# 2Retr0/GodotGaussianSplatting

Measured on NVIDIA H100. Metric: Msplats/s, higher is better.
Workload: dtype f32

## Files before the change

godotgaussiansplatting_b200/csrc/common.cuh:

```cuda
#pragma once
#include <cuda_runtime.h>
#include <stdint.h>
#include <stdio.h>

#include "../../include/gsr.h"

namespace gsr {

constexpr int TILE = 16;
constexpr int NUM_PLANES = 15;
constexpr int PROJ_THREADS = 256;

void set_last_error(const char *fmt, ...);

#define GSR_CUDA_TRY(expr)                                                                         \
    do {                                                                                           \
        cudaError_t _e = (expr);                                                                   \
        if (_e != cudaSuccess) {                                                                   \
            ::gsr::set_last_error("%s:%d: %s -> %s", __FILE__, __LINE__, #expr, cudaGetErrorString(_e)); \
            return (_e == cudaErrorMemoryAllocation) ? GSR_ERR_OOM : GSR_ERR_CUDA;                 \
        }                                                                                          \
    } while (0)

__device__ __forceinline__ float g_max(float x, float y) { return (x < y) ? y : x; }
// ... 38 lines not shown
__device__ __forceinline__ float det_pow(float x, float y) {
    if (!(x > 0.0f)) return 0.0f;
    return det_exp2(__fmul_rn(y, det_log2(x)));
}

struct FrameState {
    unsigned long long dup_total;
    uint32_t dup_sorted;
    uint32_t visible;
    int32_t last_tile_plus1;
    uint32_t overflow;
    uint32_t proj_ticket;
    uint32_t pad0;
    unsigned long long staged;
    uint32_t comp_head;
    uint32_t comp_cta_limit;
    uint32_t pad[4];
};
static_assert(sizeof(FrameState) == 64, "FrameState is one 64-byte slot of the history ring");

struct Uniforms {
    float camera_pos[3];
    float model_scale;
    int32_t dims[2];
    float time;
    float pad;
};
static_assert(sizeof(Uniforms) == 32, "uniform block must be 32 bytes");

struct SortWorkspace {
    uint32_t *hist = nullptr;
    uint32_t *status = nullptr;
    uint32_t *tickets = nullptr;
    uint32_t *alt_keys = nullptr;
    uint32_t *alt_vals = nullptr;
    uint32_t *n_dev = nullptr;
    uint64_t max_n = 0;
    uint32_t max_tiles = 0;
    int grid_hist = 0, grid_sweep_pairs = 0, grid_sweep_keys = 0;
    size_t bytes() const;
};
int sort_workspace_create(SortWorkspace &ws, uint64_t max_n, bool need_alt_buffers);
void sort_workspace_destroy(SortWorkspace &ws);
int sort_pairs_device(SortWorkspace &ws, uint32_t *keys, uint32_t *vals, const uint32_t *n_ptr, uint32_t *alt_keys,
                      uint32_t *alt_vals, cudaStream_t stream, int *launches);
uint32_t sort_tile_keys();

struct ProjectionArgs {
    const float4 *soa;
    uint64_t plane_stride;
    uint32_t num_splats;
    float vp[32];
    Uniforms u;
    float focal_base[2];
    float lim_lo[2], lim_hi[2];
    int32_t band_y0, band_y1;
    int32_t row_mod, row_rem;
    int32_t fast_reject;
    int32_t sh_bulk_min;
    int32_t fast_mode;
    float w_frob2;
    float4 *records;
    uint32_t *keys, *values;
    uint32_t capacity;
    unsigned long long *lookback;
    FrameState *frame;
};
int launch_projection(const ProjectionArgs &a, cudaStream_t stream);

constexpr int INSTANCE_FRAME_FLOATS = 32;
constexpr int INSTANCE_XFORM_FLOATS = 24;
struct InstanceDesc {
    uint64_t first;
    uint32_t count;
    uint32_t warp0;
};
struct InstanceArgs {
    const float *frame;
// ... 101 lines not shown
```

godotgaussiansplatting_b200/csrc/gsr_api.cu:

```cuda
#include <math.h>
#include <stdarg.h>
#include <stdlib.h>
#include <stddef.h>
#include <string.h>
#include <unistd.h>

#include <new>

#include "common.cuh"

namespace gsr {

static thread_local char g_last_error[512] = "";

void set_last_error(const char *fmt, ...) {
    va_list ap;
    va_start(ap, fmt);
    vsnprintf(g_last_error, sizeof g_last_error, fmt, ap);
    va_end(ap);
}

}

using namespace gsr;

constexpr int EV_PER_FRAME = 7;

struct gsr_ctx {
    int device = 0;
    uint32_t flags = 0;
    uint64_t max_splats = 0, capacity = 0, plane_stride = 0, num_splats = 0;
    uint64_t cap_stride = 0;
    cudaStream_t stream = nullptr, own_stream = nullptr;
    float4 *soa = nullptr;
    float4 *records = nullptr;
    float4 *records2 = nullptr;
    uint32_t *keys = nullptr;
    uint32_t *vals = nullptr;
    uint32_t *keys_cur = nullptr, *vals_cur = nullptr;
    float4 *records_cur = nullptr;
    cudaStream_t front_stream = nullptr;
    cudaEvent_t front_gate = nullptr;
    int overlap = -1;
    SortWorkspace sort;
    FrameState *ring = nullptr;
    FrameState *frame = nullptr;
    unsigned long long *lookback = nullptr;
    uint32_t lookback_blocks = 0;
    uint64_t frame_counter = 0;
    uint2 *bounds = nullptr;
    uint32_t *comp_order = nullptr, *comp_hint = nullptr;
    int comp_ctas_per_sm = 2, comp_order_mode = 1, comp_max_ctas = 1, comp_sparse_per_sm = 5;
    uint64_t comp_hint_key = 0;
    FrameState *pick_frame = nullptr;
    ulonglong4 *trace = nullptr;
    uint32_t *trace_count = nullptr;
    uint32_t trace_cap = 0;
    float4 *fb = nullptr, *fb_ext = nullptr;
    const float *scene_depth = nullptr;
    float *depth_out = nullptr;
    float4 *pick_strip = nullptr;
    float4 *fb2 = nullptr;
    void *stage[2] = {nullptr, nullptr};
    float4 *fb_last = nullptr;
    cudaStream_t copy_stream = nullptr;
    cudaEvent_t ev_done[2] = {nullptr, nullptr}, ev_copied[2] = {nullptr, nullptr};
    bool copied_valid[2] = {false, false};
    uint64_t async_counter = 0;
    bool peer_mode = false, peer_opened = false;
    float4 *peer_fb[2] = {nullptr, nullptr};
    uint64_t peer_counter = 0;
// ... 71 lines not shown
        return GSR_ERR_CUDA;
    }
    if (device < 0 || device >= count) {
        set_last_error("device ordinal %d out of range [0,%d)", device, count);
        return GSR_ERR_INVALID;
    }
    cudaDeviceProp prop;
    GSR_CUDA_TRY(cudaGetDeviceProperties(&prop, device));
    if (prop.major != 9 || prop.minor != 0) {
        set_last_error("device %d is sm_%d%d; libgsr is built for sm_90a only", device, prop.major, prop.minor);
        return GSR_ERR_CUDA;
    }
    return GSR_OK;
}

void group_detach(gsr_ctx *c) {
    if (c->front_stream) cudaStreamSynchronize(c->front_stream);
    if (c->stream) cudaStreamSynchronize(c->stream);
    if (c->copy_stream) cudaStreamSynchronize(c->copy_stream);
    for (int i = 0; i < c->grp.n_opened; ++i) cudaIpcCloseMemHandle(c->grp.opened[i]);
    c->grp.n_opened = 0;
    if (c->grp.world > 1) { c->row_mod = 1; c->row_rem = 0; }
    c->grp.world = 0; c->grp.rank = 0; c->grp.seq = 0; c->grp.present_rows = 0;
    c->grp.root_fb[0] = c->grp.root_fb[1] = nullptr;
}

float4 *framebuffer(gsr_ctx *c) { return c->fb_ext ? c->fb_ext : (c->fb_last ? c->fb_last : c->fb); }

void free_ctx(gsr_ctx *c) {
    if (!c) return;
    cudaSetDevice(c->device);
    if (c->stream) cudaStreamSynchronize(c->stream);
    if (c->front_stream) { cudaStreamSynchronize(c->front_stream); cudaStreamDestroy(c->front_stream); }
    cudaFree(c->soa); cudaFree(c->records); cudaFree(c->records2); cudaFree(c->keys); cudaFree(c->vals);
    sort_workspace_destroy(c->sort);
    if (c->copy_stream) cudaStreamSynchronize(c->copy_stream);
    if (c->peer_opened) { cudaIpcCloseMemHandle(c->peer_fb[0]); cudaIpcCloseMemHandle(c->peer_fb[1]); }
    cudaFree(c->stage[0]); cudaFree(c->stage[1]);
    cudaFree(c->ring); cudaFree(c->lookback); cudaFree(c->bounds); cudaFree(c->comp_order); cudaFree(c->comp_hint); cudaFree(c->pick_frame); cudaFree(c->fb); cudaFree(c->fb2); cudaFree(c->pick); cudaFree(c->staging); cudaFree(c->pick_strip);
    for (int i = 0; i < 2; ++i) { if (c->ev_done[i]) cudaEventDestroy(c->ev_done[i]); if (c->ev_copied[i]) cudaEventDestroy(c->ev_copied[i]); }
    if (c->copy_stream) cudaStreamDestroy(c->copy_stream);
    cudaFree(c->sync_word);
    for (int i = 0; i < c->grp.n_opened; ++i) cudaIpcCloseMemHandle(c->grp.opened[i]);
    cudaFree(c->grp.arena);
    cudaFree(c->unsorted_keys); cudaFree(c->unsorted_vals); cudaFree(c->trace); cudaFree(c->trace_count);
    cudaFree(c->inst.desc); cudaFree(c->inst.warps); cudaFree(c->inst.frame);
    if (c->inst.ring) cudaFreeHost(c->inst.ring);
    for (int i = 0; i < GSR_INSTANCE_RING; ++i) if (c->inst.ev[i]) cudaEventDestroy(c->inst.ev[i]);
    delete[] c->inst.range; delete[] c->inst.xf;
    if (c->ev) {
        for (int i = 0; i < GSR_HISTORY_FRAMES * EV_PER_FRAME; ++i) if (c->ev[i]) cudaEventDestroy(c->ev[i]);
        delete[] c->ev;
    }
    if (c->ev_stat) {
        for (int i = 0; i < GSR_HISTORY_FRAMES; ++i) if (c->ev_stat[i]) cudaEventDestroy(c->ev_stat[i]);
        delete[] c->ev_stat;
    }
    if (c->host_ring) cudaFreeHost(c->host_ring);
    if (c->own_stream) cudaStreamDestroy(c->own_stream);
    delete c;
}

}

extern "C" {

GSR_API const char *gsr_error_string(int code) {
// ... 40 lines not shown
#define TRY_ALLOC(ptr, bytes)                                                                      \
    do {                                                                                           \
        cudaError_t _e = cudaMalloc((void **)&(ptr), (bytes));                                     \
        if (_e != cudaSuccess) {                                                                   \
            set_last_error("cudaMalloc(%s, %llu B) -> %s", #ptr, (unsigned long long)(bytes), cudaGetErrorString(_e)); \
            free_ctx(c);                                                                           \
            return _e == cudaErrorMemoryAllocation ? GSR_ERR_OOM : GSR_ERR_CUDA;                   \
        }                                                                                          \
    } while (0)

    cudaError_t se;
    {
        int least = 0, greatest = 0;
        cudaDeviceGetStreamPriorityRange(&least, &greatest);
        se = cudaStreamCreateWithPriority(&c->own_stream, cudaStreamNonBlocking, greatest);
    }
    if (se != cudaSuccess) { set_last_error("cudaStreamCreate -> %s", cudaGetErrorString(se)); free_ctx(c); return GSR_ERR_CUDA; }
    c->stream = c->own_stream;
    se = cudaStreamCreateWithFlags(&c->copy_stream, cudaStreamNonBlocking);
    if (se == cudaSuccess) {
        int least = 0, greatest = 0;
        cudaDeviceGetStreamPriorityRange(&least, &greatest);
        se = cudaStreamCreateWithPriority(&c->front_stream, cudaStreamNonBlocking, least);
    }
    for (int i = 0; i < 2 && se == cudaSuccess; ++i) {
        se = cudaEventCreateWithFlags(&c->ev_done[i], cudaEventDisableTiming);
        if (se == cudaSuccess) se = cudaEventCreateWithFlags(&c->ev_copied[i], cudaEventDisableTiming);
    }
    if (se != cudaSuccess) { set_last_error("copy stream/events -> %s", cudaGetErrorString(se)); free_ctx(c); return GSR_ERR_CUDA; }
    TRY_ALLOC(c->soa, sizeof(float4) * NUM_PLANES * c->plane_stride);
    TRY_ALLOC(c->records, sizeof(float4) * 3ull * c->max_splats);
    TRY_ALLOC(c->records2, sizeof(float4) * 3ull * c->max_splats);
    c->cap_stride = (c->capacity + 1023ull) & ~1023ull;
    TRY_ALLOC(c->keys, sizeof(uint32_t) * 3ull * c->cap_stride);
    TRY_ALLOC(c->vals, sizeof(uint32_t) * 3ull * c->cap_stride);
    c->keys_cur = c->keys; c->vals_cur = c->vals; c->records_cur = c->records;
    c->rec_entries = c->max_splats;
    c->lookback_blocks = projection_num_blocks((uint32_t)c->max_splats);
    c->lookback_cap = c->lookback_blocks;
    TRY_ALLOC(c->ring, sizeof(FrameState) * GSR_HISTORY_FRAMES);
    TRY_ALLOC(c->lookback, sizeof(unsigned long long) * ((size_t)c->lookback_blocks + 2u * GROUP_MAX * GROUP_MAX));
    c->frame = c->ring;
    TRY_ALLOC(c->pick, sizeof(float4));
    TRY_ALLOC(c->sync_word, sizeof(int32_t));
    c->staging_splats = c->max_splats < (1ull << 18) ? c->max_splats : (1ull << 18);
    TRY_ALLOC(c->staging, sizeof(float4) * NUM_PLANES * c->staging_splats);
#undef TRY_ALLOC
    rc = sort_workspace_create(c->sort, c->capacity, false);
    if (rc) { free_ctx(c); return rc; }
    c->ev = new (std::nothrow) cudaEvent_t[GSR_HISTORY_FRAMES * EV_PER_FRAME]();
    if (!c->ev) { free_ctx(c); return GSR_ERR_OOM; }
    for (int i = 0; i < GSR_HISTORY_FRAMES * EV_PER_FRAME; ++i) {
        if (cudaEventCreate(&c->ev[i]) != cudaSuccess) { set_last_error("cudaEventCreate failed"); free_ctx(c); return GSR_ERR_CUDA; }
    }
    c->ev_stat = new (std::nothrow) cudaEvent_t[GSR_HISTORY_FRAMES]();
    if (!c->ev_stat) { free_ctx(c); return GSR_ERR_OOM; }
    for (int i = 0; i < GSR_HISTORY_FRAMES; ++i) {
        if (cudaEventCreateWithFlags(&c->ev_stat[i], cudaEventDisableTiming) != cudaSuccess) { set_last_error("cudaEventCreate failed"); free_ctx(c); return GSR_ERR_CUDA; }
    }
    if (cudaHostAlloc((void **)&c->host_ring, sizeof(FrameState) * GSR_HISTORY_FRAMES, cudaHostAllocMapped | cudaHostAllocPortable) != cudaSuccess) {
        set_last_error("cudaHostAlloc(frame mirror) failed"); c->host_ring = nullptr; free_ctx(c); return GSR_ERR_OOM;
    }
    memset(c->host_ring, 0, sizeof(FrameState) * GSR_HISTORY_FRAMES);
    cudaMemsetAsync(c->soa, 0, sizeof(float4) * NUM_PLANES * c->plane_stride, c->stream);
    cudaMemsetAsync(c->records, 0, sizeof(float4) * 3ull * c->max_splats, c->stream);
    cudaMemsetAsync(c->records2, 0, sizeof(float4) * 3ull * c->max_splats, c->stream);
    cudaMemsetAsync(c->pick, 0, sizeof(float4), c->stream);
    cudaMemsetAsync(c->sync_word, 0, sizeof(int32_t), c->stream);
    cudaMemsetAsync(c->ring, 0, sizeof(FrameState) * GSR_HISTORY_FRAMES, c->stream);
// ... 139 lines not shown
        const float tfi0 = view_proj[16 + 0], tfi1 = view_proj[16 + 5];
        const volatile float hw = (float)u.dims[0] * 0.5f, hh = (float)u.dims[1] * 0.5f;
        const volatile float f0 = hw * tfi0, f1 = hh * tfi1;
        const volatile float t0 = 1.0f / tfi0, t1 = 1.0f / tfi1;
        const volatile float n0 = -t0, n1 = -t1;
        pa.focal_base[0] = f0; pa.focal_base[1] = f1;
        pa.lim_lo[0] = n0 * 1.3f; pa.lim_lo[1] = n1 * 1.3f;
        pa.lim_hi[0] = t0 * 1.3f; pa.lim_hi[1] = t1 * 1.3f;
    }
    {
        float g[3][3];
        for (int i = 0; i < 3; ++i)
            for (int j = 0; j < 3; ++j) {
                g[i][j] = 0.0f;
                for (int r = 0; r < 3; ++r) g[i][j] += view_proj[4 * i + r] * view_proj[4 * j + r];
            }
        float nrm = 0.0f;
        for (int i = 0; i < 3; ++i) {
            float row = 0.0f;
            for (int j = 0; j < 3; ++j) row += g[i][j] < 0.0f ? -g[i][j] : g[i][j];
            nrm = row > nrm ? row : nrm;
        }
        pa.w_frob2 = nrm * 1.0001f;
    }
}

static int grow_capacity(gsr_ctx *c, uint64_t want) {
    if (want > c->capacity_max) want = c->capacity_max;
    if (want <= c->capacity) return GSR_OK;
    GSR_CUDA_TRY(cudaStreamSynchronize(c->front_stream));
    GSR_CUDA_TRY(cudaStreamSynchronize(c->stream));
    GSR_CUDA_TRY(cudaStreamSynchronize(c->copy_stream));
    c->front_gate = nullptr;
    cudaFree(c->keys); cudaFree(c->vals); c->keys = c->vals = c->keys_cur = c->vals_cur = nullptr;
    sort_workspace_destroy(c->sort);
    const bool unsorted = c->unsorted_keys != nullptr;
    cudaFree(c->unsorted_keys); cudaFree(c->unsorted_vals); c->unsorted_keys = c->unsorted_vals = nullptr;
    c->capacity = want;
    c->cap_stride = (c->capacity + 1023ull) & ~1023ull;
    GSR_CUDA_TRY(cudaMalloc((void **)&c->keys, sizeof(uint32_t) * 3ull * c->cap_stride));
    GSR_CUDA_TRY(cudaMalloc((void **)&c->vals, sizeof(uint32_t) * 3ull * c->cap_stride));
    c->keys_cur = c->keys; c->vals_cur = c->vals;
    if (unsorted) {
        GSR_CUDA_TRY(cudaMalloc((void **)&c->unsorted_keys, sizeof(uint32_t) * c->capacity));
        GSR_CUDA_TRY(cudaMalloc((void **)&c->unsorted_vals, sizeof(uint32_t) * c->capacity));
    }
    return sort_workspace_create(c->sort, c->capacity, false);
}

static int track_capacity(gsr_ctx *c) {
    if (c->flags & GSR_FLAG_STATIC_CAPACITY) return GSR_OK;
    while (c->stats_polled < c->frame_counter) {
        if (c->frame_counter - c->stats_polled > GSR_HISTORY_FRAMES) { c->stats_polled = c->frame_counter - GSR_HISTORY_FRAMES; continue; }
        const uint32_t slot = (uint32_t)(c->stats_polled % GSR_HISTORY_FRAMES);
        if (cudaEventQuery(c->ev_stat[slot]) != cudaSuccess) { cudaGetLastError(); break; }
        const uint64_t m = c->host_ring[slot].dup_total;
        if (m > c->m_high) c->m_high = m;
        c->stats_polled += 1;
    }
    if (c->m_high * 2ull > c->capacity && c->capacity < c->capacity_max) return grow_capacity(c, c->m_high * 3ull);
    return GSR_OK;
}

struct GroupFrame { uint32_t seq; int parity; int rows_local; };

static int stage_times(gsr_ctx *c, uint32_t slot, float out[5], float *front_ms) {
    cudaEvent_t *ev = c->ev + EV_PER_FRAME * slot;
    float front = 0.f, recv = 0.f;
    GSR_CUDA_TRY(cudaEventElapsedTime(&front, ev[0], ev[1]));
    GSR_CUDA_TRY(cudaEventElapsedTime(&recv, ev[2], ev[3]));
    out[0] = front + recv;
    for (int i = 1; i < 4; ++i) GSR_CUDA_TRY(cudaEventElapsedTime(&out[i], ev[2 + i], ev[3 + i]));
    out[4] = out[0] + out[1] + out[2] + out[3];
    if (front_ms) *front_ms = front;
    return GSR_OK;
// ... 4 lines not shown
static size_t arena_records_off(uint64_t cap, uint64_t max_splats, int parity) { return GROUP_FLAGS_BYTES + sizeof(uint32_t) * cap * 2 * GROUP_PHASES + sizeof(float4) * 3ull * max_splats * (size_t)parity; }
static size_t arena_bytes(uint64_t cap, uint64_t max_splats) { return arena_records_off(cap, max_splats, GROUP_PHASES); }

static GroupPeers group_peers(const gsr_ctx *c, int parity) {
    (void)parity;
    GroupPeers p;
    memset(&p, 0, sizeof p);
    p.world = c->grp.world; p.rank = c->grp.rank;
    for (int r = 0; r < c->grp.world; ++r) p.flags[r] = c->grp.flags[r];
    return p;
}

static int render_enqueue(gsr_ctx *c, const float *view_proj, const void *uniforms32, float heatmap_factor, float4 *target = nullptr,
                          const GroupFrame *gf = nullptr) {
    if (!c || !view_proj || !uniforms32) return GSR_ERR_INVALID;
    if (c->width == 0) { set_last_error("gsr_render before gsr_resize"); return GSR_ERR_STATE; }
    Uniforms u;
    memcpy(&u, uniforms32, sizeof u);
    if (u.dims[0] != c->width || u.dims[1] != c->height) {
        set_last_error("uniform dims %dx%d differ from gsr_resize %dx%d", u.dims[0], u.dims[1], c->width, c->height);
        return GSR_ERR_INVALID;
    }
    int rc = use_device(c->device);
    if (rc) return rc;
    if ((rc = track_capacity(c))) return rc;
    cudaStream_t s = c->stream;
    const bool overlap = c->overlap > 0 && c->front_stream != nullptr;
    cudaStream_t fs = overlap ? c->front_stream : s;
    int launches = 0;
    const uint32_t slot = (uint32_t)(c->frame_counter % GSR_HISTORY_FRAMES);
    c->frame = c->ring + slot;
    cudaEvent_t *ev = c->ev + EV_PER_FRAME * slot;
    const int half = (int)(c->frame_counter & 1u);
    uint32_t *keys_in = c->keys + (size_t)half * c->cap_stride, *vals_in = c->vals + (size_t)half * c->cap_stride;
    uint32_t *keys_alt = c->keys + 2ull * c->cap_stride, *vals_alt = c->vals + 2ull * c->cap_stride;
    float4 *records = half ? c->records2 : c->records;
    const uint32_t n_tiles = (uint32_t)(c->tiles_x * c->tiles_y);

    if (overlap && c->front_gate) GSR_CUDA_TRY(cudaStreamWaitEvent(fs, c->front_gate, 0));
    const bool inst = c->inst.n > 0 && !gf;
    {
        uint32_t links = projection_num_blocks((uint32_t)(inst ? c->inst.drawn : c->max_splats));
        if (gf) {
            const uint64_t first = (uint64_t)c->grp.rank * c->grp.slice;
            const uint64_t count = first < c->max_splats ? ((c->max_splats - first) < c->grp.slice ? (c->max_splats - first) : c->grp.slice) : 0;
            links = projection_scatter_blocks((uint32_t)count) * (uint32_t)c->grp.world;
        }
        if ((rc = launch_frame_clear(c->frame, c->lookback, links, overlap ? nullptr : c->bounds, overlap ? 0u : n_tiles, fs))) return rc;
        launches += 1;
    }
    GSR_CUDA_TRY(cudaEventRecord(ev[0], fs));
    if (inst) {
        const uint32_t rs = (uint32_t)(c->inst.seq % GSR_INSTANCE_RING);
        if (c->inst.ev_used[rs] && cudaEventQuery(c->inst.ev[rs]) != cudaSuccess) {
            cudaGetLastError();
            GSR_CUDA_TRY(cudaEventSynchronize(c->inst.ev[rs]));
        }
        const size_t per = (size_t)c->inst.cap * INSTANCE_XFORM_FLOATS;
        memcpy(c->inst.ring + rs * per, c->inst.xf, sizeof(float) * INSTANCE_XFORM_FLOATS * c->inst.n);
        if ((rc = launch_instance_prepare(c->inst.ring_dev + rs * per, view_proj, u.camera_pos, c->inst.n,
                                          c->inst.frame + (size_t)half * c->inst.cap * INSTANCE_FRAME_FLOATS, fs))) return rc;
        GSR_CUDA_TRY(cudaEventRecord(c->inst.ev[rs], fs));
        c->inst.ev_used[rs] = true;
        c->inst.seq += 1;
        launches += 1;
    }

    ProjectionArgs pa;
// ... 36 lines not shown
        if ((rc = launch_projection_instanced(pa, ia, fs))) return rc;
        launches += pa.num_splats ? 1 : 0;
    } else {
        if ((rc = launch_projection(pa, fs))) return rc;
        launches += pa.num_splats ? 1 : 0;
    }
    GSR_CUDA_TRY(cudaEventRecord(ev[1], fs));

    if (overlap) {
        GSR_CUDA_TRY(cudaStreamWaitEvent(s, ev[1], 0));
        if ((rc = launch_frame_clear(nullptr, nullptr, 0u, c->bounds, n_tiles, s))) return rc;
        launches += 1;
    }
    GSR_CUDA_TRY(cudaEventRecord(ev[2], s));
    if (gf) {
        const int G = c->grp.world;
        char *mine = c->grp.peer_arena[c->grp.rank];
        if ((rc = launch_group_wait_segments(c->grp.flags[c->grp.rank], gf->parity, G, gf->seq, c->grp.seg_cap, (uint32_t)c->capacity, c->frame, s))) return rc;
        if ((rc = launch_gather_segments(c->grp.flags[c->grp.rank], G, c->grp.seg_cap,
                                         reinterpret_cast<const uint32_t *>(mine + arena_rx_keys_off(c->grp.rx_capacity, gf->parity)),
                                         reinterpret_cast<const uint32_t *>(mine + arena_rx_vals_off(c->grp.rx_capacity, gf->parity)), keys_in, vals_in,
                                         c->sm_count * 8, s))) return rc;
        records = reinterpret_cast<float4 *>(mine + arena_records_off(c->grp.rx_capacity, c->max_splats, gf->parity));
        launches += 2;
    }
    c->keys_cur = keys_in; c->vals_cur = vals_in; c->records_cur = records;
    GSR_CUDA_TRY(cudaEventRecord(ev[3], s));

    if (c->keep_unsorted) {
        GSR_CUDA_TRY(cudaMemcpyAsync(c->unsorted_keys, keys_in, sizeof(uint32_t) * c->capacity, cudaMemcpyDeviceToDevice, s));
        GSR_CUDA_TRY(cudaMemcpyAsync(c->unsorted_vals, vals_in, sizeof(uint32_t) * c->capacity, cudaMemcpyDeviceToDevice, s));
    }
    const uint32_t *m_ptr = reinterpret_cast<const uint32_t *>(reinterpret_cast<const char *>(c->frame) + offsetof(FrameState, dup_sorted));
    if ((rc = sort_pairs_device(c->sort, keys_in, vals_in, m_ptr, keys_alt, vals_alt, s, &launches))) return rc;
    GSR_CUDA_TRY(cudaEventRecord(ev[4], s));

    const int sharded = fast ? 2 : ((!(c->band_y0 == 0 && c->band_y1 == c->tiles_y) || c->row_mod > 1) ? 1 : 0);
    if (fast) GSR_CUDA_TRY(cudaMemsetAsync(c->sync_word, 0, sizeof(int32_t), s));
    const int quirks = (c->flags & GSR_FLAG_FIXED_RANGES) ? 0 : 1;
    if ((rc = launch_tile_ranges(keys_in, c->frame, c->bounds, n_tiles, quirks, sharded, fast ? c->sync_word : nullptr, c->sm_count * 8, s))) return rc;
    launches += 1;
    GSR_CUDA_TRY(cudaEventRecord(ev[5], s));
    c->front_gate = ev[5];

    CompositeArgs ca;
    float4 *out_fb = c->fb_ext ? c->fb_ext : (target ? target : c->fb);
    for (int i = 0; i < 2; ++i) {
        const float4 *owned = c->peer_mode ? c->peer_fb[i] : (i ? c->fb2 : c->fb);
        if (c->copied_valid[i] && owned == out_fb) GSR_CUDA_TRY(cudaStreamWaitEvent(s, c->ev_copied[i], 0));
    }
    c->fb_last = out_fb;
    ca.records = records; ca.values = vals_in; ca.bounds = c->bounds; ca.out = out_fb;
    ca.width = c->width; ca.height = c->height; ca.tiles_x = c->tiles_x;
    {
        int first = c->band_y0 + ((c->row_rem - c->band_y0 % c->row_mod) + c->row_mod) % c->row_mod;
        int nrows = first < c->band_y1 ? (c->band_y1 - 1 - first) / c->row_mod + 1 : 0;
        ca.tile_begin = first * c->tiles_x;
        ca.row_step = c->row_mod;
        ca.num_tiles = nrows * c->tiles_x;
    }
    ca.heatmap_factor = heatmap_factor;
    ca.target_tile_id = 0xFFFFFFFFu;
    ca.pick = c->pick;
    ca.frame = c->frame; ca.count_staged = 1;
    ca.order = nullptr; ca.consumed = c->comp_hint;
    ca.ctas_per_sm = c->comp_ctas_per_sm < c->comp_max_ctas ? c->comp_ctas_per_sm : c->comp_max_ctas; ca.sm_count = c->sm_count;
    ca.contract = (c->flags & GSR_FLAG_UNCONTRACTED_BLEND) ? 0 : 1;
// ... 695 lines not shown
    if (rc) return rc;
    if ((rc = use_device(device))) return rc;
    gsr_sorter *s = new (std::nothrow) gsr_sorter();
    if (!s) return GSR_ERR_OOM;
    s->device = device;
    rc = sort_workspace_create(s->ws, max_n, true);
    if (rc == GSR_OK && (cudaEventCreate(&s->e0) != cudaSuccess || cudaEventCreate(&s->e1) != cudaSuccess)) rc = GSR_ERR_CUDA;
    if (rc) { sort_workspace_destroy(s->ws); delete s; return rc; }
    *out = s;
    return GSR_OK;
}

GSR_API int gsr_sorter_destroy(gsr_sorter *s) {
    if (!s) return GSR_OK;
    cudaSetDevice(s->device);
    cudaDeviceSynchronize();
    sort_workspace_destroy(s->ws);
    if (s->e0) cudaEventDestroy(s->e0);
    if (s->e1) cudaEventDestroy(s->e1);
    delete s;
    return GSR_OK;
}

GSR_API int gsr_sorter_sort_device(gsr_sorter *s, void *d_keys, void *d_values, uint64_t n, void *cuda_stream) {
    if (!s || (!d_keys && n)) return GSR_ERR_INVALID;
    if (n > s->ws.max_n) { set_last_error("sort of %llu exceeds sorter capacity %llu", (unsigned long long)n, (unsigned long long)s->ws.max_n); return GSR_ERR_INVALID; }
    int rc = use_device(s->device);
    if (rc) return rc;
    cudaStream_t st = (cudaStream_t)cuda_stream;
    const uint32_t n32 = (uint32_t)n;
    GSR_CUDA_TRY(cudaMemcpyAsync(s->ws.n_dev, &n32, sizeof n32, cudaMemcpyHostToDevice, st));
    GSR_CUDA_TRY(cudaEventRecord(s->e0, st));
    int launches = 0;
    rc = sort_pairs_device(s->ws, (uint32_t *)d_keys, (uint32_t *)d_values, s->ws.n_dev, s->ws.alt_keys, d_values ? s->ws.alt_vals : nullptr, st, &launches);
    if (rc) return rc;
    GSR_CUDA_TRY(cudaEventRecord(s->e1, st));
    s->timed = true;
    return GSR_OK;
}

GSR_API int gsr_sorter_last_ms(gsr_sorter *s, float *ms) {
    if (!s || !ms || !s->timed) return GSR_ERR_STATE;
    int rc = use_device(s->device);
    if (rc) return rc;
    GSR_CUDA_TRY(cudaEventSynchronize(s->e1));
    GSR_CUDA_TRY(cudaEventElapsedTime(ms, s->e0, s->e1));
    return GSR_OK;
}

GSR_API int gsr_sort_pairs_host(int32_t device, uint32_t *keys, uint32_t *values, uint64_t n) {
    if (n == 0) return GSR_OK;
    if (!keys) return GSR_ERR_INVALID;
    gsr_sorter *s = nullptr;
    int rc = gsr_sorter_create(device, n, &s);
    if (rc) return rc;
    uint32_t *dk = nullptr, *dv = nullptr;
    cudaError_t e = cudaMalloc((void **)&dk, 4 * n);
    if (e == cudaSuccess && values) e = cudaMalloc((void **)&dv, 4 * n);
    if (e == cudaSuccess) e = cudaMemcpy(dk, keys, 4 * n, cudaMemcpyHostToDevice);
    if (e == cudaSuccess && values) e = cudaMemcpy(dv, values, 4 * n, cudaMemcpyHostToDevice);
    if (e == cudaSuccess) {
        rc = gsr_sorter_sort_device(s, dk, dv, n, nullptr);
        if (rc == GSR_OK) e = cudaDeviceSynchronize();
    }
    if (e == cudaSuccess && rc == GSR_OK) e = cudaMemcpy(keys, dk, 4 * n, cudaMemcpyDeviceToHost);
    if (e == cudaSuccess && rc == GSR_OK && values) e = cudaMemcpy(values, dv, 4 * n, cudaMemcpyDeviceToHost);
    cudaFree(dk); cudaFree(dv);
// ... 7 lines not shown
```

godotgaussiansplatting_b200/csrc/radix_sort.cu:

```cuda
#include "common.cuh"

#ifndef GSR_SORT_BALLOT
#define GSR_SORT_BALLOT 1
#endif
#ifndef GSR_SORT_ATOMIC
#define GSR_SORT_ATOMIC 0
#endif

namespace gsr {

namespace {

constexpr int RADIX = 256;
constexpr uint32_t FLAG_AGG = 1u << 30;
constexpr uint32_t FLAG_PREFIX = 1u << 31;
constexpr uint32_t VAL_MASK = (1u << 30) - 1u;
constexpr int HIST_THREADS = 512;

__global__ void __launch_bounds__(HIST_THREADS) sort_hist_kernel(const uint32_t *__restrict__ keys, const uint32_t *__restrict__ n_ptr,
                                                                 uint32_t n_max, uint32_t *__restrict__ hist, uint32_t *__restrict__ status,
                                                                 uint32_t tile_keys, uint32_t max_tiles) {
    __shared__ uint32_t sh[4 * RADIX];
    const uint32_t tid = threadIdx.x;
    const uint32_t gtid = blockIdx.x * HIST_THREADS + tid;
// ... 19 lines not shown
        for (int j = 0; j < 4; ++j) {
            atomicAdd(&sh[0 * RADIX + (kk[j] & 255u)], 1u);
            atomicAdd(&sh[1 * RADIX + ((kk[j] >> 8) & 255u)], 1u);
            atomicAdd(&sh[2 * RADIX + ((kk[j] >> 16) & 255u)], 1u);
            atomicAdd(&sh[3 * RADIX + (kk[j] >> 24)], 1u);
        }
    }
    for (uint32_t i = (n4 << 2) + gtid; i < n; i += gsize) {
        const uint32_t k = keys[i];
        atomicAdd(&sh[0 * RADIX + (k & 255u)], 1u);
        atomicAdd(&sh[1 * RADIX + ((k >> 8) & 255u)], 1u);
        atomicAdd(&sh[2 * RADIX + ((k >> 16) & 255u)], 1u);
        atomicAdd(&sh[3 * RADIX + (k >> 24)], 1u);
    }
    __syncthreads();
    for (uint32_t i = tid; i < 4 * RADIX; i += HIST_THREADS) {
        const uint32_t v = sh[i];
        if (v) atomicAdd(&hist[i], v);
    }
}

__device__ __forceinline__ uint32_t lane_id() { return threadIdx.x & 31u; }

__device__ __forceinline__ uint32_t warp_incl_scan(uint32_t v) {
    const uint32_t lane = lane_id();
#pragma unroll
    for (int o = 1; o < 32; o <<= 1) {
        const uint32_t t = __shfl_up_sync(0xffffffffu, v, o);
        if (lane >= (uint32_t)o) v += t;
    }
    return v;
}

template <int THREADS, int ITEMS, bool PAIRS>
__global__ void __launch_bounds__(THREADS, 1024 / THREADS) onesweep_kernel(const uint32_t *__restrict__ keys_in, uint32_t *__restrict__ keys_out,
                                                           const uint32_t *__restrict__ vals_in, uint32_t *__restrict__ vals_out,
                                                           const uint32_t *__restrict__ n_ptr, uint32_t n_max,
                                                           const uint32_t *__restrict__ hist,
                                                           uint32_t *status,
                                                           uint32_t *ticket, int shift) {
    static_assert(THREADS >= RADIX && THREADS % 32 == 0, "need one thread per digit");
    constexpr int WARPS = THREADS / 32;
    constexpr uint32_t TILE_KEYS = THREADS * ITEMS;
#ifndef GSR_CPU_EMU
    extern __shared__ uint32_t smem[];
#else
    __shared__ uint32_t smem[WARPS * RADIX + 2 * TILE_KEYS];
#endif
    uint32_t *s_whist = smem;
    uint32_t *s_keys = s_whist + WARPS * RADIX;
    uint32_t *s_vals = s_keys + TILE_KEYS;
    __shared__ uint32_t s_gbase[RADIX];
    __shared__ uint32_t s_dstart[RADIX];
    __shared__ uint32_t s_base[RADIX];
    __shared__ uint32_t s_wtot[RADIX / 32];
    __shared__ uint32_t s_tile;

    const uint32_t tid = threadIdx.x, lane = tid & 31u, warp = tid >> 5;
    uint32_t n = *n_ptr;
    n = n < n_max ? n : n_max;
    const uint32_t num_tiles = (n + TILE_KEYS - 1) / TILE_KEYS;

    {
        uint32_t v = 0, incl = 0;
        if (tid < RADIX) {
            v = hist[tid];
            incl = warp_incl_scan(v);
            if (lane == 31) s_wtot[warp] = incl;
        }
        __syncthreads();
        if (tid < RADIX) {
            uint32_t off = 0;
            for (uint32_t w = 0; w < warp; ++w) off += s_wtot[w];
            s_gbase[tid] = off + incl - v;
        }
    }

    while (true) {
        __syncthreads();
        if (tid == 0) s_tile = atomicAdd(ticket, 1u);
        for (uint32_t i = tid; i < WARPS * RADIX; i += THREADS) s_whist[i] = 0u;
        __syncthreads();
        const uint32_t tile = s_tile;
        if (tile >= num_tiles) break;

        const uint32_t tile_base = tile * TILE_KEYS;
        const uint32_t my_base = tile_base + warp * (32u * ITEMS) + lane;
        const bool full = (tile_base + TILE_KEYS) <= n;
        uint32_t key[ITEMS], val[ITEMS], rank[ITEMS];
        if (full) {
#pragma unroll
            for (int i = 0; i < ITEMS; ++i) key[i] = keys_in[my_base + i * 32u];
            if (PAIRS) {
#pragma unroll
                for (int i = 0; i < ITEMS; ++i) val[i] = vals_in[my_base + i * 32u];
            }
        } else {
#pragma unroll
            for (int i = 0; i < ITEMS; ++i) {
                const uint32_t idx = my_base + i * 32u;
                key[i] = idx < n ? keys_in[idx] : 0xFFFFFFFFu;
                if (PAIRS) val[i] = idx < n ? vals_in[idx] : 0u;
            }
        }

        uint32_t *wh = s_whist + warp * RADIX;
        const uint32_t lt_mask = (1u << lane) - 1u;
#if GSR_SORT_ATOMIC
        uint32_t old[ITEMS];
#pragma unroll
        for (int i = 0; i < ITEMS; ++i) {
            const uint32_t d = (key[i] >> shift) & 255u;
#if GSR_SORT_BALLOT
            uint32_t mask = 0xffffffffu;
#pragma unroll
            for (int b = 0; b < 8; ++b) {
                const bool bit = (d >> b) & 1u;
                const uint32_t bal = __ballot_sync(0xffffffffu, bit);
                mask &= bit ? bal : ~bal;
            }
#else
            const uint32_t mask = __match_any_sync(0xffffffffu, d);
#endif
            rank[i] = (uint32_t)__popc(mask & lt_mask) | ((uint32_t)(__ffs(mask) - 1) << 8);
            old[i] = 0u;
            if ((mask & lt_mask) == 0u) old[i] = atomicAdd(&wh[d], (uint32_t)__popc(mask));
            __syncwarp();
        }
#pragma unroll
        for (int i = 0; i < ITEMS; ++i) {
            const uint32_t meta = rank[i];
            const uint32_t prev = __shfl_sync(0xffffffffu, old[i], (int)(meta >> 8));
            rank[i] = prev + (meta & 255u);
        }
#else
// ... 19 lines not shown
        }
#endif
        __syncthreads();

        uint32_t agg = 0, incl = 0;
        if (tid < RADIX) {
            uint32_t sum = 0;
#pragma unroll 4
            for (int w = 0; w < WARPS; ++w) {
                const uint32_t c = s_whist[w * RADIX + tid];
                s_whist[w * RADIX + tid] = sum;
                sum += c;
            }
            agg = sum;
            volatile uint32_t *st = status + (size_t)tile * RADIX + tid;
            *st = (tile == 0 ? FLAG_PREFIX : FLAG_AGG) | agg;
            incl = warp_incl_scan(agg);
            if (lane == 31) s_wtot[warp] = incl;
        }
        __syncthreads();
        uint32_t dstart = 0;
        if (tid < RADIX) {
            uint32_t off = 0;
            for (uint32_t w = 0; w < warp; ++w) off += s_wtot[w];
            dstart = off + incl - agg;
            s_dstart[tid] = dstart;
        }
        __syncthreads();

#pragma unroll
        for (int i = 0; i < ITEMS; ++i) {
            const uint32_t d = (key[i] >> shift) & 255u;
            const uint32_t pos = s_dstart[d] + wh[d] + rank[i];
            s_keys[pos] = key[i];
            if (PAIRS) s_vals[pos] = val[i];
        }

        if (tid < RADIX) {
            uint32_t excl = 0;
            if (tile > 0) {
                int64_t t = (int64_t)tile - 1;
                while (true) {
                    volatile uint32_t *st = status + (size_t)t * RADIX + tid;
                    uint32_t v;
                    do { v = *st; } while ((v & (FLAG_AGG | FLAG_PREFIX)) == 0u);
                    excl += v & VAL_MASK;
                    if (v & FLAG_PREFIX) break;
                    --t;
                }
                volatile uint32_t *mine = status + (size_t)tile * RADIX + tid;
                *mine = FLAG_PREFIX | ((excl + agg) & VAL_MASK);
            }
            s_base[tid] = s_gbase[tid] + excl - dstart;
        }
        __syncthreads();

        const uint32_t tile_n = (n - tile_base) < TILE_KEYS ? (n - tile_base) : TILE_KEYS;
        for (uint32_t idx = tid; idx < tile_n; idx += THREADS) {
            const uint32_t k = s_keys[idx];
            const uint32_t dst = s_base[(k >> shift) & 255u] + idx;
            keys_out[dst] = k;
            if (PAIRS) vals_out[dst] = s_vals[idx];
        }
    }
}

struct SweepConfig { int threads, items; };
#ifndef GSR_SORT_THREADS
#define GSR_SORT_THREADS 512
#endif
#ifndef GSR_SORT_ITEMS
#define GSR_SORT_ITEMS 10
#endif
constexpr int SWEEP_THREADS = GSR_SORT_THREADS;
constexpr int SWEEP_ITEMS = GSR_SORT_ITEMS;
constexpr uint32_t SWEEP_TILE = SWEEP_THREADS * SWEEP_ITEMS;

template <bool PAIRS>
constexpr size_t sweep_smem() {
    return sizeof(uint32_t) * ((SWEEP_THREADS / 32) * RADIX + SWEEP_TILE * (PAIRS ? 2 : 1));
}

}

#ifndef GSR_CPU_EMU

int preload_sort_kernels() {
    cudaFuncAttributes fa;
    GSR_CUDA_TRY(cudaFuncGetAttributes(&fa, sort_hist_kernel));
    GSR_CUDA_TRY(cudaFuncGetAttributes(&fa, onesweep_kernel<SWEEP_THREADS, SWEEP_ITEMS, true>));
    GSR_CUDA_TRY(cudaFuncGetAttributes(&fa, onesweep_kernel<SWEEP_THREADS, SWEEP_ITEMS, false>));
    return GSR_OK;
}
size_t SortWorkspace::bytes() const {
    return sizeof(uint32_t) * (4 * RADIX + 8) + sizeof(uint32_t) * 4ull * max_tiles * RADIX + (alt_keys ? 8ull * max_n : 0);
}

int sort_workspace_create(SortWorkspace &ws, uint64_t max_n, bool need_alt_buffers) {
    if (max_n == 0 || max_n >= (1ull << 30)) {
        set_last_error("sorter: max_n=%llu outside [1, 2^30)", (unsigned long long)max_n);
        return GSR_ERR_INVALID;
    }
    ws.max_n = max_n;
    ws.max_tiles = (uint32_t)((max_n + SWEEP_TILE - 1) / SWEEP_TILE);
    GSR_CUDA_TRY(cudaMalloc(&ws.hist, sizeof(uint32_t) * (4 * RADIX + 8)));
    ws.tickets = ws.hist + 4 * RADIX;
    ws.n_dev = ws.hist + 4 * RADIX + 4;
    GSR_CUDA_TRY(cudaMalloc(&ws.status, sizeof(uint32_t) * 4ull * ws.max_tiles * RADIX));
    if (need_alt_buffers) {
        GSR_CUDA_TRY(cudaMalloc(&ws.alt_keys, sizeof(uint32_t) * max_n));
        GSR_CUDA_TRY(cudaMalloc(&ws.alt_vals, sizeof(uint32_t) * max_n));
    }
    int dev = 0;
    GSR_CUDA_TRY(cudaGetDevice(&dev));
    int sm_count = 0;
    GSR_CUDA_TRY(cudaDeviceGetAttribute(&sm_count, cudaDevAttrMultiProcessorCount, dev));
    auto kp = onesweep_kernel<SWEEP_THREADS, SWEEP_ITEMS, true>;
    auto kk = onesweep_kernel<SWEEP_THREADS, SWEEP_ITEMS, false>;
    GSR_CUDA_TRY(cudaFuncSetAttribute(kp, cudaFuncAttributeMaxDynamicSharedMemorySize, (int)sweep_smem<true>()));
    GSR_CUDA_TRY(cudaFuncSetAttribute(kk, cudaFuncAttributeMaxDynamicSharedMemorySize, (int)sweep_smem<false>()));
    int occ_p = 0, occ_k = 0;
    GSR_CUDA_TRY(cudaOccupancyMaxActiveBlocksPerMultiprocessor(&occ_p, kp, SWEEP_THREADS, sweep_smem<true>()));
    GSR_CUDA_TRY(cudaOccupancyMaxActiveBlocksPerMultiprocessor(&occ_k, kk, SWEEP_THREADS, sweep_smem<false>()));
    if (occ_p < 1 || occ_k < 1) {
        set_last_error("sorter: onesweep kernel does not fit on an SM");
        return GSR_ERR_CUDA;
    }
    auto cap_grid = [&](int g) { return (int)((uint32_t)g < ws.max_tiles ? (uint32_t)g : ws.max_tiles); };
    ws.grid_sweep_pairs = cap_grid(sm_count * occ_p);
    ws.grid_sweep_keys = cap_grid(sm_count * occ_k);
    ws.grid_hist = sm_count * 4;
    return GSR_OK;
}

void sort_workspace_destroy(SortWorkspace &ws) {
    cudaFree(ws.hist);
    cudaFree(ws.status);
    cudaFree(ws.alt_keys);
    cudaFree(ws.alt_vals);
    ws = SortWorkspace();
}

int sort_pairs_device(SortWorkspace &ws, uint32_t *keys, uint32_t *vals, const uint32_t *n_ptr, uint32_t *alt_keys,
                      uint32_t *alt_vals, cudaStream_t stream, int *launches) {
    const uint32_t n_max = (uint32_t)ws.max_n;
    GSR_CUDA_TRY(cudaMemsetAsync(ws.hist, 0, sizeof(uint32_t) * (4 * RADIX + 4), stream));
    sort_hist_kernel<<<ws.grid_hist, HIST_THREADS, 0, stream>>>(keys, n_ptr, n_max, ws.hist, ws.status, SWEEP_TILE, ws.max_tiles);
    uint32_t *kin = keys, *kout = alt_keys, *vin = vals, *vout = alt_vals;
    for (int pass = 0; pass < 4; ++pass) {
        uint32_t *st = ws.status + (size_t)pass * ws.max_tiles * RADIX;
        if (vals) {
            onesweep_kernel<SWEEP_THREADS, SWEEP_ITEMS, true><<<ws.grid_sweep_pairs, SWEEP_THREADS, sweep_smem<true>(), stream>>>(
                kin, kout, vin, vout, n_ptr, n_max, ws.hist + pass * RADIX, st, ws.tickets + pass, 8 * pass);
        } else {
            onesweep_kernel<SWEEP_THREADS, SWEEP_ITEMS, false><<<ws.grid_sweep_keys, SWEEP_THREADS, sweep_smem<false>(), stream>>>(
                kin, kout, nullptr, nullptr, n_ptr, n_max, ws.hist + pass * RADIX, st, ws.tickets + pass, 8 * pass);
        }
        uint32_t *t = kin; kin = kout; kout = t;
        t = vin; vin = vout; vout = t;
    }
    GSR_CUDA_TRY(cudaGetLastError());
    if (launches) *launches += 5;
    return GSR_OK;
}

uint32_t sort_tile_keys() { return SWEEP_TILE; }
#endif

}
```

Baseline: 3371.

## Use interleaved key-value pairs for intermediate radix sort passes

The onesweep radix sort now keeps keys and values interleaved as uint2 in shared memory and in the intermediate global buffers, so the middle passes read and scatter one 8-byte element instead of two separate 4-byte arrays. The first pass unpacks from separate arrays and the last pass writes separate arrays back. Key and value buffers are merged into one allocation so the second packed buffer can alias the current frame's key/value region. Items per thread rise from 10 to 12, which changes the tile size and the shared memory footprint.

```diff
diff --git a/godotgaussiansplatting_b200/csrc/common.cuh b/godotgaussiansplatting_b200/csrc/common.cuh
--- a/godotgaussiansplatting_b200/csrc/common.cuh
+++ b/godotgaussiansplatting_b200/csrc/common.cuh
@@ -94,18 +94,17 @@
     uint32_t *hist = nullptr;
     uint32_t *status = nullptr;
     uint32_t *tickets = nullptr;
-    uint32_t *alt_keys = nullptr;
-    uint32_t *alt_vals = nullptr;
+    uint2 *packed = nullptr;
     uint32_t *n_dev = nullptr;
     uint64_t max_n = 0;
     uint32_t max_tiles = 0;
     int grid_hist = 0, grid_sweep_pairs = 0, grid_sweep_keys = 0;
     size_t bytes() const;
 };
-int sort_workspace_create(SortWorkspace &ws, uint64_t max_n, bool need_alt_buffers);
+int sort_workspace_create(SortWorkspace &ws, uint64_t max_n, bool need_packed_buffers);
 void sort_workspace_destroy(SortWorkspace &ws);
-int sort_pairs_device(SortWorkspace &ws, uint32_t *keys, uint32_t *vals, const uint32_t *n_ptr, uint32_t *alt_keys,
-                      uint32_t *alt_vals, cudaStream_t stream, int *launches);
+int sort_pairs_device(SortWorkspace &ws, uint32_t *keys, uint32_t *vals, const uint32_t *n_ptr, uint2 *packed_a, uint2 *packed_b,
+                      cudaStream_t stream, int *launches);
 uint32_t sort_tile_keys();
 
 struct ProjectionArgs {
diff --git a/godotgaussiansplatting_b200/csrc/gsr_api.cu b/godotgaussiansplatting_b200/csrc/gsr_api.cu
--- a/godotgaussiansplatting_b200/csrc/gsr_api.cu
+++ b/godotgaussiansplatting_b200/csrc/gsr_api.cu
@@ -35,8 +35,7 @@
     float4 *soa = nullptr;
     float4 *records = nullptr;
     float4 *records2 = nullptr;
-    uint32_t *keys = nullptr;
-    uint32_t *vals = nullptr;
+    uint32_t *pairs = nullptr;
     uint32_t *keys_cur = nullptr, *vals_cur = nullptr;
     float4 *records_cur = nullptr;
     cudaStream_t front_stream = nullptr;
@@ -174,7 +173,7 @@
     cudaSetDevice(c->device);
     if (c->stream) cudaStreamSynchronize(c->stream);
     if (c->front_stream) { cudaStreamSynchronize(c->front_stream); cudaStreamDestroy(c->front_stream); }
-    cudaFree(c->soa); cudaFree(c->records); cudaFree(c->records2); cudaFree(c->keys); cudaFree(c->vals);
+    cudaFree(c->soa); cudaFree(c->records); cudaFree(c->records2); cudaFree(c->pairs);
     sort_workspace_destroy(c->sort);
     if (c->copy_stream) cudaStreamSynchronize(c->copy_stream);
     if (c->peer_opened) { cudaIpcCloseMemHandle(c->peer_fb[0]); cudaIpcCloseMemHandle(c->peer_fb[1]); }
@@ -281,9 +280,8 @@
     TRY_ALLOC(c->records, sizeof(float4) * 3ull * c->max_splats);
     TRY_ALLOC(c->records2, sizeof(float4) * 3ull * c->max_splats);
     c->cap_stride = (c->capacity + 1023ull) & ~1023ull;
-    TRY_ALLOC(c->keys, sizeof(uint32_t) * 3ull * c->cap_stride);
-    TRY_ALLOC(c->vals, sizeof(uint32_t) * 3ull * c->cap_stride);
-    c->keys_cur = c->keys; c->vals_cur = c->vals; c->records_cur = c->records;
+    TRY_ALLOC(c->pairs, sizeof(uint32_t) * 6ull * c->cap_stride);
+    c->keys_cur = c->pairs; c->vals_cur = c->pairs + c->cap_stride; c->records_cur = c->records;
     c->rec_entries = c->max_splats;
     c->lookback_blocks = projection_num_blocks((uint32_t)c->max_splats);
     c->lookback_cap = c->lookback_blocks;
@@ -489,15 +487,14 @@
     GSR_CUDA_TRY(cudaStreamSynchronize(c->stream));
     GSR_CUDA_TRY(cudaStreamSynchronize(c->copy_stream));
     c->front_gate = nullptr;
-    cudaFree(c->keys); cudaFree(c->vals); c->keys = c->vals = c->keys_cur = c->vals_cur = nullptr;
+    cudaFree(c->pairs); c->pairs = c->keys_cur = c->vals_cur = nullptr;
     sort_workspace_destroy(c->sort);
     const bool unsorted = c->unsorted_keys != nullptr;
     cudaFree(c->unsorted_keys); cudaFree(c->unsorted_vals); c->unsorted_keys = c->unsorted_vals = nullptr;
     c->capacity = want;
     c->cap_stride = (c->capacity + 1023ull) & ~1023ull;
-    GSR_CUDA_TRY(cudaMalloc((void **)&c->keys, sizeof(uint32_t) * 3ull * c->cap_stride));
-    GSR_CUDA_TRY(cudaMalloc((void **)&c->vals, sizeof(uint32_t) * 3ull * c->cap_stride));
-    c->keys_cur = c->keys; c->vals_cur = c->vals;
+    GSR_CUDA_TRY(cudaMalloc((void **)&c->pairs, sizeof(uint32_t) * 6ull * c->cap_stride));
+    c->keys_cur = c->pairs; c->vals_cur = c->pairs + c->cap_stride;
     if (unsorted) {
         GSR_CUDA_TRY(cudaMalloc((void **)&c->unsorted_keys, sizeof(uint32_t) * c->capacity));
         GSR_CUDA_TRY(cudaMalloc((void **)&c->unsorted_vals, sizeof(uint32_t) * c->capacity));
@@ -568,8 +565,8 @@
     c->frame = c->ring + slot;
     cudaEvent_t *ev = c->ev + EV_PER_FRAME * slot;
     const int half = (int)(c->frame_counter & 1u);
-    uint32_t *keys_in = c->keys + (size_t)half * c->cap_stride, *vals_in = c->vals + (size_t)half * c->cap_stride;
-    uint32_t *keys_alt = c->keys + 2ull * c->cap_stride, *vals_alt = c->vals + 2ull * c->cap_stride;
+    uint32_t *keys_in = c->pairs + 2ull * half * c->cap_stride, *vals_in = keys_in + c->cap_stride;
+    uint2 *packed_alt = reinterpret_cast<uint2 *>(c->pairs + 4ull * c->cap_stride);
     float4 *records = half ? c->records2 : c->records;
     const uint32_t n_tiles = (uint32_t)(c->tiles_x * c->tiles_y);
 
@@ -672,7 +669,7 @@
         GSR_CUDA_TRY(cudaMemcpyAsync(c->unsorted_vals, vals_in, sizeof(uint32_t) * c->capacity, cudaMemcpyDeviceToDevice, s));
     }
     const uint32_t *m_ptr = reinterpret_cast<const uint32_t *>(reinterpret_cast<const char *>(c->frame) + offsetof(FrameState, dup_sorted));
-    if ((rc = sort_pairs_device(c->sort, keys_in, vals_in, m_ptr, keys_alt, vals_alt, s, &launches))) return rc;
+    if ((rc = sort_pairs_device(c->sort, keys_in, vals_in, m_ptr, packed_alt, reinterpret_cast<uint2 *>(keys_in), s, &launches))) return rc;
     GSR_CUDA_TRY(cudaEventRecord(ev[4], s));
 
     const int sharded = fast ? 2 : ((!(c->band_y0 == 0 && c->band_y1 == c->tiles_y) || c->row_mod > 1) ? 1 : 0);
@@ -1434,7 +1431,7 @@
     GSR_CUDA_TRY(cudaMemcpyAsync(s->ws.n_dev, &n32, sizeof n32, cudaMemcpyHostToDevice, st));
     GSR_CUDA_TRY(cudaEventRecord(s->e0, st));
     int launches = 0;
-    rc = sort_pairs_device(s->ws, (uint32_t *)d_keys, (uint32_t *)d_values, s->ws.n_dev, s->ws.alt_keys, d_values ? s->ws.alt_vals : nullptr, st, &launches);
+    rc = sort_pairs_device(s->ws, (uint32_t *)d_keys, (uint32_t *)d_values, s->ws.n_dev, s->ws.packed, s->ws.packed + s->ws.max_n, st, &launches);
     if (rc) return rc;
     GSR_CUDA_TRY(cudaEventRecord(s->e1, st));
     s->timed = true;
diff --git a/godotgaussiansplatting_b200/csrc/radix_sort.cu b/godotgaussiansplatting_b200/csrc/radix_sort.cu
--- a/godotgaussiansplatting_b200/csrc/radix_sort.cu
+++ b/godotgaussiansplatting_b200/csrc/radix_sort.cu
@@ -75,24 +75,26 @@
     return v;
 }
 
-template <int THREADS, int ITEMS, bool PAIRS>
+template <int THREADS, int ITEMS, bool PAIRS, bool PACKED_IN = false, bool PACKED_OUT = false>
 __global__ void __launch_bounds__(THREADS, 1024 / THREADS) onesweep_kernel(const uint32_t *__restrict__ keys_in, uint32_t *__restrict__ keys_out,
                                                            const uint32_t *__restrict__ vals_in, uint32_t *__restrict__ vals_out,
                                                            const uint32_t *__restrict__ n_ptr, uint32_t n_max,
                                                            const uint32_t *__restrict__ hist,
                                                            uint32_t *status,
-                                                           uint32_t *ticket, int shift) {
+                                                           uint32_t *ticket, int shift,
+                                                           const uint2 *__restrict__ pairs_in = nullptr, uint2 *__restrict__ pairs_out = nullptr) {
     static_assert(THREADS >= RADIX && THREADS % 32 == 0, "need one thread per digit");
+    static_assert(PAIRS || (!PACKED_IN && !PACKED_OUT), "keys only has no packed layout");
     constexpr int WARPS = THREADS / 32;
     constexpr uint32_t TILE_KEYS = THREADS * ITEMS;
 #ifndef GSR_CPU_EMU
-    extern __shared__ uint32_t smem[];
+    extern __shared__ __align__(16) uint32_t smem[];
 #else
-    __shared__ uint32_t smem[WARPS * RADIX + 2 * TILE_KEYS];
+    alignas(16) __shared__ uint32_t smem[WARPS * RADIX + 2 * TILE_KEYS];
 #endif
     uint32_t *s_whist = smem;
     uint32_t *s_keys = s_whist + WARPS * RADIX;
-    uint32_t *s_vals = s_keys + TILE_KEYS;
+    uint2 *s_pairs = reinterpret_cast<uint2 *>(s_keys);
     __shared__ uint32_t s_gbase[RADIX];
     __shared__ uint32_t s_dstart[RADIX];
     __shared__ uint32_t s_base[RADIX];
@@ -132,18 +134,33 @@
         const bool full = (tile_base + TILE_KEYS) <= n;
         uint32_t key[ITEMS], val[ITEMS], rank[ITEMS];
         if (full) {
-#pragma unroll
-            for (int i = 0; i < ITEMS; ++i) key[i] = keys_in[my_base + i * 32u];
-            if (PAIRS) {
-#pragma unroll
-                for (int i = 0; i < ITEMS; ++i) val[i] = vals_in[my_base + i * 32u];
+            if (PACKED_IN) {
+#pragma unroll
+                for (int i = 0; i < ITEMS; ++i) {
+                    const uint2 p = pairs_in[my_base + i * 32u];
+                    key[i] = p.x;
+                    val[i] = p.y;
+                }
+            } else {
+#pragma unroll
+                for (int i = 0; i < ITEMS; ++i) key[i] = keys_in[my_base + i * 32u];
+                if (PAIRS) {
+#pragma unroll
+                    for (int i = 0; i < ITEMS; ++i) val[i] = vals_in[my_base + i * 32u];
+                }
             }
         } else {
 #pragma unroll
             for (int i = 0; i < ITEMS; ++i) {
                 const uint32_t idx = my_base + i * 32u;
-                key[i] = idx < n ? keys_in[idx] : 0xFFFFFFFFu;
-                if (PAIRS) val[i] = idx < n ? vals_in[idx] : 0u;
+                if (PACKED_IN) {
+                    const uint2 p = idx < n ? pairs_in[idx] : make_uint2(0xFFFFFFFFu, 0u);
+                    key[i] = p.x;
+                    val[i] = p.y;
+                } else {
+                    key[i] = idx < n ? keys_in[idx] : 0xFFFFFFFFu;
+                    if (PAIRS) val[i] = idx < n ? vals_in[idx] : 0u;
+                }
             }
         }
 
@@ -229,8 +246,8 @@
         for (int i = 0; i < ITEMS; ++i) {
             const uint32_t d = (key[i] >> shift) & 255u;
             const uint32_t pos = s_dstart[d] + wh[d] + rank[i];
-            s_keys[pos] = key[i];
-            if (PAIRS) s_vals[pos] = val[i];
+            if (PAIRS) s_pairs[pos] = make_uint2(key[i], val[i]);
+            else s_keys[pos] = key[i];
         }
 
         if (tid < RADIX) {
@@ -253,11 +270,23 @@
         __syncthreads();
 
         const uint32_t tile_n = (n - tile_base) < TILE_KEYS ? (n - tile_base) : TILE_KEYS;
-        for (uint32_t idx = tid; idx < tile_n; idx += THREADS) {
-            const uint32_t k = s_keys[idx];
-            const uint32_t dst = s_base[(k >> shift) & 255u] + idx;
-            keys_out[dst] = k;
-            if (PAIRS) vals_out[dst] = s_vals[idx];
+        if (PAIRS) {
+            for (uint32_t idx = tid; idx < tile_n; idx += THREADS) {
+                const uint2 p = s_pairs[idx];
+                const uint32_t dst = s_base[(p.x >> shift) & 255u] + idx;
+                if (PACKED_OUT) {
+                    pairs_out[dst] = p;
+                } else {
+                    keys_out[dst] = p.x;
+                    vals_out[dst] = p.y;
+                }
+            }
+        } else {
+            for (uint32_t idx = tid; idx < tile_n; idx += THREADS) {
+                const uint32_t k = s_keys[idx];
+                const uint32_t dst = s_base[(k >> shift) & 255u] + idx;
+                keys_out[dst] = k;
+            }
         }
     }
 }
@@ -267,7 +296,7 @@
 #define GSR_SORT_THREADS 512
 #endif
 #ifndef GSR_SORT_ITEMS
-#define GSR_SORT_ITEMS 10
+#define GSR_SORT_ITEMS 12
 #endif
 constexpr int SWEEP_THREADS = GSR_SORT_THREADS;
 constexpr int SWEEP_ITEMS = GSR_SORT_ITEMS;
@@ -278,6 +307,10 @@
     return sizeof(uint32_t) * ((SWEEP_THREADS / 32) * RADIX + SWEEP_TILE * (PAIRS ? 2 : 1));
 }
 
+template <bool PACKED_IN, bool PACKED_OUT>
+constexpr auto sweep_pairs_kernel = onesweep_kernel<SWEEP_THREADS, SWEEP_ITEMS, true, PACKED_IN, PACKED_OUT>;
+constexpr auto sweep_keys_kernel = onesweep_kernel<SWEEP_THREADS, SWEEP_ITEMS, false, false, false>;
+
 }
 
 #ifndef GSR_CPU_EMU
@@ -285,15 +318,17 @@
 int preload_sort_kernels() {
     cudaFuncAttributes fa;
     GSR_CUDA_TRY(cudaFuncGetAttributes(&fa, sort_hist_kernel));
-    GSR_CUDA_TRY(cudaFuncGetAttributes(&fa, onesweep_kernel<SWEEP_THREADS, SWEEP_ITEMS, true>));
-    GSR_CUDA_TRY(cudaFuncGetAttributes(&fa, onesweep_kernel<SWEEP_THREADS, SWEEP_ITEMS, false>));
+    GSR_CUDA_TRY(cudaFuncGetAttributes(&fa, sweep_pairs_kernel<false, true>));
+    GSR_CUDA_TRY(cudaFuncGetAttributes(&fa, sweep_pairs_kernel<true, true>));
+    GSR_CUDA_TRY(cudaFuncGetAttributes(&fa, sweep_pairs_kernel<true, false>));
+    GSR_CUDA_TRY(cudaFuncGetAttributes(&fa, sweep_keys_kernel));
     return GSR_OK;
 }
 size_t SortWorkspace::bytes() const {
-    return sizeof(uint32_t) * (4 * RADIX + 8) + sizeof(uint32_t) * 4ull * max_tiles * RADIX + (alt_keys ? 8ull * max_n : 0);
-}
-
-int sort_workspace_create(SortWorkspace &ws, uint64_t max_n, bool need_alt_buffers) {
+    return sizeof(uint32_t) * (4 * RADIX + 8) + sizeof(uint32_t) * 4ull * max_tiles * RADIX + (packed ? 16ull * max_n : 0);
+}
+
+int sort_workspace_create(SortWorkspace &ws, uint64_t max_n, bool need_packed_buffers) {
     if (max_n == 0 || max_n >= (1ull << 30)) {
         set_last_error("sorter: max_n=%llu outside [1, 2^30)", (unsigned long long)max_n);
         return GSR_ERR_INVALID;
@@ -304,21 +339,20 @@
     ws.tickets = ws.hist + 4 * RADIX;
     ws.n_dev = ws.hist + 4 * RADIX + 4;
     GSR_CUDA_TRY(cudaMalloc(&ws.status, sizeof(uint32_t) * 4ull * ws.max_tiles * RADIX));
-    if (need_alt_buffers) {
-        GSR_CUDA_TRY(cudaMalloc(&ws.alt_keys, sizeof(uint32_t) * max_n));
-        GSR_CUDA_TRY(cudaMalloc(&ws.alt_vals, sizeof(uint32_t) * max_n));
-    }
+    if (need_packed_buffers) GSR_CUDA_TRY(cudaMalloc(&ws.packed, sizeof(uint2) * 2ull * max_n));
     int dev = 0;
     GSR_CUDA_TRY(cudaGetDevice(&dev));
     int sm_count = 0;
     GSR_CUDA_TRY(cudaDeviceGetAttribute(&sm_count, cudaDevAttrMultiProcessorCount, dev));
-    auto kp = onesweep_kernel<SWEEP_THREADS, SWEEP_ITEMS, true>;
-    auto kk = onesweep_kernel<SWEEP_THREADS, SWEEP_ITEMS, false>;
-    GSR_CUDA_TRY(cudaFuncSetAttribute(kp, cudaFuncAttributeMaxDynamicSharedMemorySize, (int)sweep_smem<true>()));
-    GSR_CUDA_TRY(cudaFuncSetAttribute(kk, cudaFuncAttributeMaxDynamicSharedMemorySize, (int)sweep_smem<false>()));
-    int occ_p = 0, occ_k = 0;
-    GSR_CUDA_TRY(cudaOccupancyMaxActiveBlocksPerMultiprocessor(&occ_p, kp, SWEEP_THREADS, sweep_smem<true>()));
-    GSR_CUDA_TRY(cudaOccupancyMaxActiveBlocksPerMultiprocessor(&occ_k, kk, SWEEP_THREADS, sweep_smem<false>()));
+    int occ_p = 1 << 30, occ_k = 0;
+    for (auto kp : {sweep_pairs_kernel<false, true>, sweep_pairs_kernel<true, true>, sweep_pairs_kernel<true, false>}) {
+        int occ = 0;
+        GSR_CUDA_TRY(cudaFuncSetAttribute(kp, cudaFuncAttributeMaxDynamicSharedMemorySize, (int)sweep_smem<true>()));
+        GSR_CUDA_TRY(cudaOccupancyMaxActiveBlocksPerMultiprocessor(&occ, kp, SWEEP_THREADS, sweep_smem<true>()));
+        occ_p = occ < occ_p ? occ : occ_p;
+    }
+    GSR_CUDA_TRY(cudaFuncSetAttribute(sweep_keys_kernel, cudaFuncAttributeMaxDynamicSharedMemorySize, (int)sweep_smem<false>()));
+    GSR_CUDA_TRY(cudaOccupancyMaxActiveBlocksPerMultiprocessor(&occ_k, sweep_keys_kernel, SWEEP_THREADS, sweep_smem<false>()));
     if (occ_p < 1 || occ_k < 1) {
         set_last_error("sorter: onesweep kernel does not fit on an SM");
         return GSR_ERR_CUDA;
@@ -333,28 +367,34 @@
 void sort_workspace_destroy(SortWorkspace &ws) {
     cudaFree(ws.hist);
     cudaFree(ws.status);
-    cudaFree(ws.alt_keys);
-    cudaFree(ws.alt_vals);
+    cudaFree(ws.packed);
     ws = SortWorkspace();
 }
 
-int sort_pairs_device(SortWorkspace &ws, uint32_t *keys, uint32_t *vals, const uint32_t *n_ptr, uint32_t *alt_keys,
-                      uint32_t *alt_vals, cudaStream_t stream, int *launches) {
+int sort_pairs_device(SortWorkspace &ws, uint32_t *keys, uint32_t *vals, const uint32_t *n_ptr, uint2 *packed_a, uint2 *packed_b,
+                      cudaStream_t stream, int *launches) {
     const uint32_t n_max = (uint32_t)ws.max_n;
     GSR_CUDA_TRY(cudaMemsetAsync(ws.hist, 0, sizeof(uint32_t) * (4 * RADIX + 4), stream));
     sort_hist_kernel<<<ws.grid_hist, HIST_THREADS, 0, stream>>>(keys, n_ptr, n_max, ws.hist, ws.status, SWEEP_TILE, ws.max_tiles);
-    uint32_t *kin = keys, *kout = alt_keys, *vin = vals, *vout = alt_vals;
+    const int smem_p = (int)sweep_smem<true>(), smem_k = (int)sweep_smem<false>();
     for (int pass = 0; pass < 4; ++pass) {
-        uint32_t *st = ws.status + (size_t)pass * ws.max_tiles * RADIX;
+        const uint32_t *h = ws.hist + pass * RADIX;
+        uint32_t *st = ws.status + (size_t)pass * ws.max_tiles * RADIX, *tk = ws.tickets + pass;
+        const int sh = 8 * pass;
         if (vals) {
-            onesweep_kernel<SWEEP_THREADS, SWEEP_ITEMS, true><<<ws.grid_sweep_pairs, SWEEP_THREADS, sweep_smem<true>(), stream>>>(
-                kin, kout, vin, vout, n_ptr, n_max, ws.hist + pass * RADIX, st, ws.tickets + pass, 8 * pass);
+            const int g = ws.grid_sweep_pairs;
+            if (pass == 0)
+                sweep_pairs_kernel<false, true><<<g, SWEEP_THREADS, smem_p, stream>>>(keys, nullptr, vals, nullptr, n_ptr, n_max, h, st, tk, sh, nullptr, packed_a);
+            else if (pass == 3)
+                sweep_pairs_kernel<true, false><<<g, SWEEP_THREADS, smem_p, stream>>>(nullptr, keys, nullptr, vals, n_ptr, n_max, h, st, tk, sh, packed_a, nullptr);
+            else
+                sweep_pairs_kernel<true, true><<<g, SWEEP_THREADS, smem_p, stream>>>(nullptr, nullptr, nullptr, nullptr, n_ptr, n_max, h, st, tk, sh,
+                                                                                    pass == 1 ? packed_a : packed_b, pass == 1 ? packed_b : packed_a);
         } else {
-            onesweep_kernel<SWEEP_THREADS, SWEEP_ITEMS, false><<<ws.grid_sweep_keys, SWEEP_THREADS, sweep_smem<false>(), stream>>>(
-                kin, kout, nullptr, nullptr, n_ptr, n_max, ws.hist + pass * RADIX, st, ws.tickets + pass, 8 * pass);
-        }
-        uint32_t *t = kin; kin = kout; kout = t;
-        t = vin; vin = vout; vout = t;
+            uint32_t *alt = reinterpret_cast<uint32_t *>(packed_a);
+            sweep_keys_kernel<<<ws.grid_sweep_keys, SWEEP_THREADS, smem_k, stream>>>(pass & 1 ? alt : keys, pass & 1 ? keys : alt, nullptr, nullptr, n_ptr,
+                                                                                     n_max, h, st, tk, sh, nullptr, nullptr);
+        }
     }
     GSR_CUDA_TRY(cudaGetLastError());
     if (launches) *launches += 5;
```

Result: faster. 3457, median of 6 (+2.6%).
